# yuliangguo/OmniFusion

Measured on AMD Instinct MI355X. Metric: panoramas/sec at 512x1024 ERP, N=18 256^2 patches; equi2pers+pers2equi GB/s vs HBM peak, higher is better.
Workload: dtype f16x3 (fp16 hi/lo pairs, fp32 accumulate: fp32-class); 1 GPU; cfg2/cfg4 shard: 8 panoramas/GPU/step, 512x1024 ERP, fov 80, nrows 4 (18 patches); full single-pass spherical_fusion forward (confidence=True) at patch size 128 — the only size the reference network exists at (SURVEY 0.1); random-init weights (seed 42); inputs resident in HBM; resample pair at 18x256^2 reported in roofline_resample; per_gpu_batch=8, global_batch=8, parallelism=image-sharded x1, execution=3 forwards in flight per GPU on 3 streams (spherical_fusion.pipelined)

## Files before the change

omnifusion_amd/csrc/omni_conv_up2_taps.hip:

```cpp
#include <stdint.h>
#include "omni_up2_tapsum.h"

namespace {

struct TapsArgs {
    const void* src;
    const void* wt;
    const float* bias;
    void* dst;
    int M, Hl, Cout, act;
};

constexpr int TAP_BYTES = 32 * 256;

__device__ __forceinline__ void wait_taps_in_flight(int n)
{
    if (n >= 16) wait_vm<16>();
    else if (n == 14) wait_vm<14>();
    else if (n == 12) wait_vm<12>();
    else if (n == 10) wait_vm<10>();
    else if (n == 8) wait_vm<8>();
    else if (n == 6) wait_vm<6>();
    else if (n == 4) wait_vm<4>();
    else if (n == 2) wait_vm<2>();
    else wait_vm<0>();
}

template <int WL, int ROWS, int HALO>
__global__ __launch_bounds__(256, 1) void up2_taps_fused_kernel(TapsArgs a)
{
    static_assert((WL == 32 && ROWS == 8 && HALO == 1) || (WL == 16 && ROWS == 16 && HALO == 0), "bands of 8 rows of 32-wide maps, or whole 16 x 16 maps");
    constexpr int SROWS = ROWS + 2 * HALO, P = SROWS * WL, NF = P / 32, NFW = (NF + 3) / 4;
    constexpr int W_BYTES = 9 * TAP_BYTES, CH_BYTES = P * 128, ROW_BYTES = WL * 128;
    static_assert(P % 32 == 0 && ROWS * WL == 256, "whole fragments; one (column, channel quad) thread per eight rows");
    __shared__ __attribute__((aligned(1024))) unsigned char lds[W_BYTES + 2 * CH_BYTES];
    static_assert(sizeof(lds) <= 160 * 1024, "one block per CU");

    const int t = threadIdx.x, lane = t & 63;
    const int wave = __builtin_amdgcn_readfirstlane(t >> 6);
    const int ntn = a.Cout >> 5, nb = a.Hl / ROWS;
    int bid = blockIdx.x;
    const int tile_n = bid % ntn; bid /= ntn;
    const int band = bid % nb; const int m = bid / nb;
    const int r0 = band * ROWS, col0 = tile_n * 32, sbase = r0 - HALO;
    const int Hl = a.Hl;

    auto frag = [&](int fi) { const int f = wave + 4 * fi; return f < NF ? f : wave + 4; };
    h8v xh[NFW][4], xl[NFW][4];
#pragma unroll
    for (int fi = 0; fi < NFW; ++fi) {
        const int f = frag(fi);
        {
            const int p = f * 32 + (lane & 31), sr = p / WL, cx = p - sr * WL;
            const int row = min(max(sbase + sr, 0), Hl - 1);
            const unsigned char* sp = (const unsigned char*)a.src + ((size_t)(m * Hl + row) * WL + cx) * 256 + (lane >> 5) * 16;
#pragma unroll
            for (int kc = 0; kc < 4; ++kc) {
                xh[fi][kc] = *reinterpret_cast<const h8v*>(sp + (kc >> 1) * 128 + (kc & 1) * 32);
                xl[fi][kc] = *reinterpret_cast<const h8v*>(sp + (kc >> 1) * 128 + 64 + (kc & 1) * 32);
            }
        }
    }
    {
        const rsrc_t rsw = make_rsrc(a.wt, (size_t)9 * a.Cout * 256);
#pragma unroll
        for (int s = 0; s < 9; ++s) {
            const int tp = tap_at(s);
#pragma unroll
            for (int k = 0; k < 2; ++k) {
                const int i = wave + 4 * k, row = 4 * i + (lane >> 4), piece = (lane & 15) ^ (row & 15);
                dma16(rsw, lds + tp * TAP_BYTES + i * 1024, ((tp * a.Cout + col0 + row) * 16 + piece) * 16, 0);
            }
        }
    }
    const int wfo = (lane & 31) * 256 + (((lane >> 5) ^ (lane & 15)) * 16);

    const int quad = t & 7, j = (t >> 3) & (WL - 1);
    const int ib = WL == 32 ? 0 : 8 * (wave >> 1);
    int coff[3];
#pragma unroll
    for (int c = 0; c < 3; ++c) coff[c] = tapsum_col_off(min(max(j - 1 + c, 0), WL - 1), quad);
    float hx[4], lx[4];
    tapsum_col_weights<WL>(j, hx, lx);
    const TapsumRowW wy = tapsum_row_weights(r0 + ib == 0, r0 + ib + 7 == Hl - 1);

    f4v out[8][2][2];
    f4v S[8][2];

    wait_taps_in_flight(16);
    __builtin_amdgcn_s_barrier();
    asm volatile("" ::: "memory");

    auto tap = [&]<int s>() {
        constexpr int tp = tap_at(s), ky = tp / 3, kx = tp - 3 * ky;
        unsigned char* chunk = lds + W_BYTES + (s & 1) * CH_BYTES;
        {
            const unsigned char* wb = lds + tp * TAP_BYTES;
            h8v wh[4], wl[4];
#pragma unroll
            for (int kc = 0; kc < 4; ++kc) {
                const int K = 8 * (kc >> 1) + 2 * (kc & 1);
                wh[kc] = *reinterpret_cast<const h8v*>(wb + (wfo ^ (K * 16)));
                wl[kc] = *reinterpret_cast<const h8v*>(wb + (wfo ^ ((K + 4) * 16)));
            }
#pragma unroll
            for (int fi = 0; fi < NFW; ++fi) {
                const int f = frag(fi);
                {
                    f16v acc = (f16v)(0.0f), acc1 = (f16v)(0.0f);
#pragma unroll
                    for (int kc = 0; kc < 4; ++kc) {
                        acc  = __builtin_amdgcn_mfma_f32_32x32x16_f16(wh[kc], xh[fi][kc], acc, 0, 0, 0);
                        acc1 = __builtin_amdgcn_mfma_f32_32x32x16_f16(wl[kc], xh[fi][kc], acc1, 0, 0, 0);
                        acc1 = __builtin_amdgcn_mfma_f32_32x32x16_f16(wh[kc], xl[fi][kc], acc1, 0, 0, 0);
                    }
                    const int px = f * 32 + (lane & 31);
                    tapsum_park(acc1, acc, chunk + px * 128, (px >> 1) & 3, lane >> 5);
                }
                __builtin_amdgcn_sched_barrier(0);
            }
        }
        if (s < 8) wait_taps_in_flight(2 * (7 - s));
        wait_lds_reads();
        __builtin_amdgcn_s_barrier();
        asm volatile("" ::: "memory");
        tapsum_vertical<8, ky, ROW_BYTES>(S, chunk, r0 + ib, sbase, Hl, coff[1], wy);
        if constexpr (ky == 2) {
            unsigned char* other = lds + W_BYTES + ((s & 1) ^ 1) * CH_BYTES;
            tapsum_put<8, 0, ROW_BYTES>(S, other, ib, coff[1]);
            wait_lds_reads();
            __builtin_amdgcn_s_barrier();
            asm volatile("" ::: "memory");
            tapsum_put<8, 1, ROW_BYTES>(S, chunk, ib, coff[1]);
            __builtin_amdgcn_sched_barrier(0);
            tapsum_horizontal<8, kx, 0, ROW_BYTES>(out, S, other, ib, coff[0], coff[2], hx, lx);
            wait_lds_reads();
            __builtin_amdgcn_s_barrier();
            asm volatile("" ::: "memory");
            tapsum_horizontal<8, kx, 1, ROW_BYTES>(out, S, chunk, ib, coff[0], coff[2], hx, lx);
        }
    };
    tap.template operator()<0>(); tap.template operator()<1>(); tap.template operator()<2>();
    tap.template operator()<3>(); tap.template operator()<4>(); tap.template operator()<5>();
    tap.template operator()<6>(); tap.template operator()<7>(); tap.template operator()<8>();

    f4v bv = (f4v)(0.0f);
    if (a.bias) bv = *reinterpret_cast<const f4v*>(a.bias + col0 + quad * 4);
    const int Ho = 2 * Hl, Wo = 2 * WL;
#pragma unroll
    for (int it = 0; it < 8; ++it)
#pragma unroll
        for (int ay = 0; ay < 2; ++ay)
#pragma unroll
            for (int bx = 0; bx < 2; ++bx) {
                f4v o = out[it][ay][bx] + bv;
                if (a.act == OMNI_ACT_RELU) { o.x = fmaxf(o.x, 0.f); o.y = fmaxf(o.y, 0.f); o.z = fmaxf(o.z, 0.f); o.w = fmaxf(o.w, 0.f); }
                const int oy = 2 * (r0 + ib + it) + ay, ox = 2 * j + bx;
                act_store4<true>(a.dst, (((size_t)m * Ho + oy) * Wo + ox) * a.Cout + col0 + quad * 4, o);
            }
}

}

OMNI_SH_OVERFLOW_ACCESSOR(omni_sh_overflow_up2_taps)

extern "C" int omni_conv3x3_up2_taps_sh_f16x3(const void* src, const void* wt16t, const float* bias, void* dst, int fmt,
                                              int M, int Hl, int Wl, int C, int Cout, int act, omni_stream_t stream)
{
    if (!src || !wt16t || !dst) OMNI_FAIL(OMNI_ERR_INVALID, "omni_conv3x3_up2_taps_sh: null pointer");
    if (M <= 0 || Hl <= 0 || Wl <= 0 || C <= 0 || C % 32 || Cout <= 0 || Cout % 32) OMNI_FAIL(OMNI_ERR_INVALID, "omni_conv3x3_up2_taps_sh: bad shape (channels must be multiples of 32)");
    if ((uintptr_t)src % 16 || (uintptr_t)wt16t % 16 || (uintptr_t)bias % 16 || (uintptr_t)dst % 16) OMNI_FAIL(OMNI_ERR_INVALID, "omni_conv3x3_up2_taps_sh: tensors must be 16-byte aligned");
    const bool bands = Wl == 32 && Hl % 8 == 0, image = Wl == 16 && Hl == 16;
    if ((fmt & ~4) != 1 || C != 64 || Cout != 64 || !(bands || image) || (act != OMNI_ACT_NONE && act != OMNI_ACT_RELU))
        OMNI_FAIL(OMNI_ERR_UNSUPPORTED, "omni_conv3x3_up2_taps_sh: serves f16x3 with an SH result, 64 -> 64 channels, Wl = 32 with Hl % 8 == 0 or 16 x 16 maps, no activation or ReLU");
    if ((long long)M * Hl * Wl * 4 >= (1ll << 31)) OMNI_FAIL(OMNI_ERR_UNSUPPORTED, "omni_conv3x3_up2_taps_sh: tensor too large for 32-bit indices");
    TapsArgs a;
    a.src = src; a.wt = wt16t; a.bias = bias; a.dst = dst; a.M = M; a.Hl = Hl; a.Cout = Cout; a.act = act;
    const unsigned ntn = (unsigned)(Cout / 32);
    if (bands) hipLaunchKernelGGL((up2_taps_fused_kernel<32, 8, 1>), dim3((unsigned)M * (unsigned)(Hl / 8) * ntn), dim3(256), 0, (hipStream_t)stream, a);
    else       hipLaunchKernelGGL((up2_taps_fused_kernel<16, 16, 0>), dim3((unsigned)M * ntn), dim3(256), 0, (hipStream_t)stream, a);
    OMNI_HIP(hipGetLastError());
    return OMNI_OK;
}
```

omnifusion_amd/csrc/omni_geometry.hip:

```cpp
#include <math.h>
#include <stdlib.h>
#include <string.h>
#include <mutex>
#include <vector>
#include <memory>

#include "omni_internal.h"

static thread_local std::string g_err;
void omni_set_error(const std::string& msg) { g_err = msg; }
extern "C" const char* omni_last_error(void) { return g_err.c_str(); }
extern "C" int omni_version(void) { return OMNI_VERSION; }

namespace {
struct OptName { const char* name; const char* env; int OmniOptions::* field; int dflt; };
const OptName kOpts[] = {
    {"conv_sh_tile", "OMNI_CONV_SH_TILE", &OmniOptions::conv_sh_tile, -1},
    {"conv_nohalo", "OMNI_CONV_NOHALO", &OmniOptions::conv_nohalo, 0},
    {"conv_halo_th", "OMNI_CONV_HALO_TH", &OmniOptions::conv_halo_th, 4},
    {"conv_big_blocks", "OMNI_CONV_BIG_BLOCKS", &OmniOptions::conv_big_blocks, 128},
    {"conv_halo_bn_lat", "OMNI_CONV_HALO_BN_LAT", &OmniOptions::conv_halo_bn_lat, 32},
    {"conv_deep_loaders", "OMNI_CONV_DEEP_LOADERS", &OmniOptions::conv_deep_loaders, 1},
    {"conv_halo_up2_bn_lat", "OMNI_CONV_HALO_UP2_BN_LAT", &OmniOptions::conv_halo_up2_bn_lat, 64},
    {"conv_halo_bn", "OMNI_CONV_HALO_BN", &OmniOptions::conv_halo_bn, 64},
    {"conv_img", "OMNI_CONV_IMG", &OmniOptions::conv_img, 1},
    {"conv_nodeep", "OMNI_CONV_NODEEP", &OmniOptions::conv_nodeep, 0},
    {"conv_pingpong", "OMNI_CONV_PINGPONG", &OmniOptions::conv_pingpong, 1},
    {"conv_pm", "OMNI_CONV_PM", &OmniOptions::conv_pm, 1},
    {"conv_noxcd", "OMNI_CONV_NOXCD", &OmniOptions::conv_noxcd, 0},
    {"conv_wt_major", "OMNI_CONV_WT_MAJOR", &OmniOptions::conv_wt_major, 1},
    {"conv_stem_pc", "OMNI_CONV_STEM_PC", &OmniOptions::conv_stem_pc, 1},
    {"conv_epi_lds", "OMNI_CONV_EPI_LDS", &OmniOptions::conv_epi_lds, 1},
    {"conv_up2_persist", "OMNI_CONV_UP2_PERSIST", &OmniOptions::conv_up2_persist, 1},
    {"conv_up2_heads_taps", "OMNI_CONV_UP2_HEADS_TAPS", &OmniOptions::conv_up2_heads_taps, 1},
    {"splitk_max", "OMNI_SPLITK_MAX", &OmniOptions::splitk_max, 0},
    {"e2p_gather", "OMNI_E2P_GATHER", &OmniOptions::e2p_gather, 0},
    {"e2p_notab", "OMNI_E2P_NOTAB", &OmniOptions::e2p_notab, 0},
    {"e2p_verbose", "OMNI_E2P_VERBOSE", &OmniOptions::e2p_verbose, 0},
    {"e2p_bwd_simple", "OMNI_E2P_BWD_SIMPLE", &OmniOptions::e2p_bwd_simple, 0},
    {"p2e_bwd_simple", "OMNI_P2E_BWD_SIMPLE", &OmniOptions::p2e_bwd_simple, 0},
    {"bwd_table_mb", "OMNI_BWD_TABLE_MB", &OmniOptions::bwd_table_mb, 1024},
    {"bwd_wide", "OMNI_BWD_WIDE", &OmniOptions::bwd_wide, 1},
    {"bwd_lmax", "OMNI_BWD_LMAX", &OmniOptions::bwd_lmax, 0},
    {"bwd_chunk", "OMNI_BWD_CHUNK", &OmniOptions::bwd_chunk, 0},
    {"p2e_gather", "OMNI_P2E_GATHER", &OmniOptions::p2e_gather, 0},
    {"e2p_nbuf", "OMNI_E2P_NBUF", &OmniOptions::e2p_nbuf, 0},
    {"e2p_slot_kb", "OMNI_E2P_SLOT_KB", &OmniOptions::e2p_slot_kb, 6},
    {"e2p_tile_h", "OMNI_E2P_TILE_H", &OmniOptions::e2p_tile_h, 0},
    {"e2p_ref_lds", "OMNI_E2P_REF_LDS", &OmniOptions::e2p_ref_lds, 1},
    {"e2p_store", "OMNI_E2P_STORE", &OmniOptions::e2p_store, 1},
    {"e2p_slots", "OMNI_E2P_SLOTS", &OmniOptions::e2p_slots, 0},
    {"e2p_split", "OMNI_E2P_SPLIT", &OmniOptions::e2p_split, 0},
    {"e2p_full", "OMNI_E2P_FULL", &OmniOptions::e2p_full, -1},
    {"e2p_fb_planes", "OMNI_E2P_FB_PLANES", &OmniOptions::e2p_fb_planes, 0},
    {"e2p_fb_pos", "OMNI_E2P_FB_POS", &OmniOptions::e2p_fb_pos, 0},
    {"e2p_region", "OMNI_E2P_REGION", &OmniOptions::e2p_region, 0},
    {"p2e_band", "OMNI_P2E_BAND", &OmniOptions::p2e_band, 0},
    {"p2e_nbuf", "OMNI_P2E_NBUF", &OmniOptions::p2e_nbuf, 0},
    {"p2e_lds_kb", "OMNI_P2E_LDS_KB", &OmniOptions::p2e_lds_kb, 0},
    {"p2e_planes", "OMNI_P2E_PLANES", &OmniOptions::p2e_planes, 0},
    {"p2e_walk", "OMNI_P2E_WALK", &OmniOptions::p2e_walk, 1},
    {"p2e_tile8", "OMNI_P2E_TILE8", &OmniOptions::p2e_tile8, 1},
    {"p2e_store", "OMNI_P2E_STORE", &OmniOptions::p2e_store, 1},
    {"fv_bwd_lds", "OMNI_FV_BWD_LDS", &OmniOptions::fv_bwd_lds, 1},
    {"geom_cache_max", "OMNI_GEOM_CACHE_MAX", &OmniOptions::geom_cache_max, 16},
    {"chamfer_split", "OMNI_CHAMFER_SPLIT", &OmniOptions::chamfer_split, 1},
    {"augment_lut", "OMNI_AUGMENT_LUT", &OmniOptions::augment_lut, 1},
    {"conv_halo2", "OMNI_CONV_HALO2", &OmniOptions::conv_halo2, 1},
    {"conv_wgrad_rows", "OMNI_CONV_WGRAD_ROWS", &OmniOptions::conv_wgrad_rows, 0},
};
}

OmniOptions& omni_options()
{
    static OmniOptions o = [] {
        OmniOptions v;
        for (const OptName& k : kOpts) {
            const char* e = getenv(k.env);
            v.*(k.field) = e ? (*e ? atoi(e) : 1) : k.dflt;
        }
        return v;
    }();
    return o;
}

int omni_num_cus()
{
    static int cus[64] = {0};
    int dev = 0;
    if (hipGetDevice(&dev) != hipSuccess || dev < 0 || dev >= 64) return 256;
    if (cus[dev] == 0) {
        int n = 0;
        cus[dev] = (hipDeviceGetAttribute(&n, hipDeviceAttributeMultiprocessorCount, dev) == hipSuccess && n > 0) ? n : 256;
    }
    return cus[dev];
}

extern "C" int omni_set_option(const char* name, int value)
{
    if (!name) OMNI_FAIL(OMNI_ERR_INVALID, "omni_set_option: null name");
    for (const OptName& k : kOpts)
        if (strcmp(k.name, name) == 0) { omni_options().*(k.field) = value; return OMNI_OK; }
    OMNI_FAIL(OMNI_ERR_INVALID, std::string("omni_set_option: unknown option '") + name + "'");
}

extern "C" int omni_get_option(const char* name, int* value)
{
    if (!name || !value) OMNI_FAIL(OMNI_ERR_INVALID, "omni_get_option: null argument");
    for (const OptName& k : kOpts)
        if (strcmp(k.name, name) == 0) { *value = omni_options().*(k.field); return OMNI_OK; }
    OMNI_FAIL(OMNI_ERR_INVALID, std::string("omni_get_option: unknown option '") + name + "'");
}

#ifdef OMNI_DEBUG_BUILD
int omni_debug_bits(const char* env_name) { const char* d = getenv(env_name); return d ? atoi(d) : 0; }
static long long* g_omni_trace = nullptr;
long long* omni_debug_trace_buf() { return g_omni_trace; }
extern "C" int omni_debug_set_trace(long long* buf) { g_omni_trace = buf; return OMNI_OK; }
#endif

namespace {
struct Preset { int nr; const int* cols; const double* phis; };

bool preset(int nrows, int which, Preset& p)
{
    static const int c4[] = {3, 6, 6, 3};            static const double p4[] = {-67.5, -22.5, 22.5, 67.5};
    static const int c6[] = {3, 8, 12, 12, 8, 3};    static const double p6[] = {-75.2, -45.93, -15.72, 15.72, 45.93, 75.2};
    static const int c3[] = {3, 4, 3};               static const double p3e[] = {-60, 0, 60};
    static const double p3p[] = {-59.6, 0, 59.6};
    static const int c5[] = {3, 6, 8, 6, 3};         static const double p5[] = {-72.2, -36.1, 0, 36.1, 72.2};
    switch (nrows) {
    case 4: p = {4, c4, p4}; return true;
    case 6: p = {6, c6, p6}; return true;
    case 3: p = {3, c3, which ? p3p : p3e}; return true;
    case 5: p = {5, c5, p5}; return true;
    default: return false;
    }
}

int centers(int nrows, int which, float* lam0, float* phi1, float* center_p)
{
    Preset p;
    if (!preset(nrows, which, p)) return -1;
    const float PI_F = (float)M_PI, PI_2_F = (float)(M_PI * 0.5);
    int n = 0;
    for (int i = 0; i < p.nr; ++i)
        for (int j = 0; j < p.cols[i]; ++j) {
            double ti = 360.0 / p.cols[i];
            double tc = j * ti + ti / 2;
            float cx = (float)tc / 360.0f;
            float cy = ((float)p.phis[i] + 90.0f) / 180.0f;
            float px = cx * 2.0f - 1.0f, py = cy * 2.0f - 1.0f;
            if (center_p) { center_p[2 * n] = px; center_p[2 * n + 1] = py; }
            if (lam0) lam0[n] = px * PI_F;
            if (phi1) phi1[n] = py * PI_2_F;
            ++n;
        }
    return n;
}

void fill_tab(PatchTab& t, int nrows, int which)
{
    float lam[OMNI_MAX_PATCH], phi[OMNI_MAX_PATCH];
    t.N = centers(nrows, which, lam, phi, nullptr);
    for (int n = 0; n < t.N; ++n) {
        t.lam0[n] = lam[n];
        t.slam[n] = (float)sin((double)lam[n]); t.clam[n] = (float)cos((double)lam[n]);
        t.sphi[n] = (float)sin((double)phi[n]); t.cphi[n] = (float)cos((double)phi[n]);
    }
}

float linspace_f(float start, float end, int steps, int idx)
{
    if (steps == 1) return start;
    float step = (end - start) / (float)(steps - 1);
    int half = steps / 2;
    return idx < half ? fmaf(step, (float)idx, start) : fmaf(-step, (float)(steps - idx - 1), end);
}
}

extern "C" int omni_num_patches(int nrows) { return centers(nrows, 0, nullptr, nullptr, nullptr); }

extern "C" int omni_patch_centers(int nrows, int which, float* center_p_host)
{
    if (!center_p_host) OMNI_FAIL(OMNI_ERR_INVALID, "omni_patch_centers: null output");
    int n = centers(nrows, which, nullptr, nullptr, center_p_host);
    if (n < 0) OMNI_FAIL(OMNI_ERR_INVALID, "unsupported nrows " + std::to_string(nrows) + " (presets: 3,4,5,6)");
    return OMNI_OK;
}

extern "C" int omni_geometry_create(omni_geometry_t** out, int nrows, float fov_h, float fov_w,
                                    int ph, int pw, int H, int W, omni_stream_t stream_)
{
    hipStream_t stream = (hipStream_t)stream_;
    if (!out) OMNI_FAIL(OMNI_ERR_INVALID, "omni_geometry_create: null out");
    if (omni_num_patches(nrows) < 0)
        OMNI_FAIL(OMNI_ERR_INVALID, "unsupported nrows " + std::to_string(nrows) + " (presets: 3,4,5,6)");
    if (ph < 1 || pw < 1 || H < 0 || W < 0 || ph > 32768 || pw > 32768 || H > 32768 || W > 32768)
        OMNI_FAIL(OMNI_ERR_INVALID, "omni_geometry_create: bad patch/ERP size");
    if (!(fov_h > 0.f) || !(fov_w > 0.f)) OMNI_FAIL(OMNI_ERR_INVALID, "omni_geometry_create: fov must be > 0");

    std::unique_ptr<omni_geometry> g(new omni_geometry());
    OMNI_HIP(hipGetDevice(&g->device));
    g->nrows = nrows; g->fov_h = fov_h; g->fov_w = fov_w; g->ph = ph; g->pw = pw; g->H = H; g->W = W;
    fill_tab(g->e2p, nrows, 0);
    fill_tab(g->p2e, nrows, 1);
    g->N = g->e2p.N;
    centers(nrows, 0, nullptr, nullptr, g->center_p);
    g->row_trig = nullptr; g->col_trig = nullptr; g->cand = nullptr; g->ntx = (W + 63) / 64;
    g->e2p_fb_tiles = nullptr; g->e2p_nfb = 0; g->e2p_ixy = nullptr; g->e2p_ts = 32;
    for (auto& t : g->p2e_tiles) { t.ent = nullptr; t.ord = nullptr; t.walk = nullptr; t.nslots = 0; t.max_chunks = 0; t.max_cand = 0; t.ok = 0; t.sum_chunks = 0; }
    for (auto& t : g->e2p_boxes) { t.ent = nullptr; t.fb = nullptr; t.order = nullptr; t.norder = 0; t.nfb = 0; t.max_chunks = 0; t.ok = 0; t.tw = t.th = t.tx = t.ty = 0; }
    g->p2e_tx = g->p2e_ty = 0; g->pinned = 0;
    g->p2e_bwd_box = nullptr; g->p2e_rden = nullptr; g->p2e_btx = g->p2e_bty = g->p2e_bwd_ok = 0;
    g->p2e_bwd_ids = nullptr; g->p2e_bwd_nsmall = g->p2e_bwd_nbig = 0;
    g->e2p_bwd_box = nullptr; g->e2p_bwd_ids = nullptr; g->e2p_bwd_nsmall = g->e2p_bwd_nbig = g->e2p_gtx = g->e2p_gty = g->e2p_bwd_ok = 0;

    if (H > 0 && W > 0) {
        const float PI_F = (float)M_PI, PI_2_F = (float)(M_PI * 0.5);
        std::vector<float2> rt(H), ct(W);
        for (int i = 0; i < H; ++i) { double a = (double)linspace_f(-PI_2_F, PI_2_F, H, i); rt[i] = make_float2((float)sin(a), (float)cos(a)); }
        for (int j = 0; j < W; ++j) { double a = (double)linspace_f(-PI_F, PI_F, W, j);     ct[j] = make_float2((float)sin(a), (float)cos(a)); }
        OMNI_HIP(hipMalloc((void**)&g->row_trig, sizeof(float2) * H));
        OMNI_HIP(hipMalloc((void**)&g->col_trig, sizeof(float2) * W));
        OMNI_HIP(hipMalloc((void**)&g->cand, sizeof(unsigned long long) * (size_t)H * g->ntx));
        OMNI_HIP(hipMemcpy(g->row_trig, rt.data(), sizeof(float2) * H, hipMemcpyHostToDevice));
        OMNI_HIP(hipMemcpy(g->col_trig, ct.data(), sizeof(float2) * W, hipMemcpyHostToDevice));
        int rc = omni_p2e_build_candidates(g.get(), stream);
        if (rc == OMNI_OK) rc = omni_p2e_build_tiles(g.get(), stream);
        if (rc == OMNI_OK) rc = omni_e2p_build_tileflags(g.get(), stream);
        if (rc == OMNI_OK) rc = omni_e2p_build_boxes(g.get(), stream);
        if (rc != OMNI_OK) { omni_geometry_destroy(g.release()); return rc; }
    }
    *out = g.release();
    return OMNI_OK;
}

int omni_bwd_workspace(omni_geometry* g, hipStream_t stream, size_t bytes, float** out)
{
    std::lock_guard<std::mutex> lk(g->ws_mu);
    omni_geometry::Ws* w = nullptr;
    for (auto& x : g->bwd_ws)
        if (x.stream == stream) {
            if (x.bytes >= bytes) { *out = x.ptr; return OMNI_OK; }
            w = &x;
        }
    hipStreamCaptureStatus cs = hipStreamCaptureStatusNone;
    if (stream && hipStreamIsCapturing(stream, &cs) == hipSuccess && cs == hipStreamCaptureStatusActive)
        OMNI_FAIL(OMNI_ERR_UNSUPPORTED, "backward: first use of a batch size on this geometry and stream while the stream is being captured (run the shape once before capturing)");
    if (!w || g->pinned) { g->bwd_ws.push_back({stream, nullptr, 0}); w = &g->bwd_ws.back(); }
    if (w->ptr) { OMNI_HIP(hipStreamSynchronize(stream)); OMNI_HIP(hipFree(w->ptr)); w->ptr = nullptr; w->bytes = 0; }
    OMNI_HIP(hipMalloc((void**)&w->ptr, bytes));
    w->bytes = bytes; *out = w->ptr;
    return OMNI_OK;
}

extern "C" void omni_geometry_destroy(omni_geometry_t* g)
{
    if (!g) return;
    if (g->row_trig) (void)hipFree(g->row_trig);
    if (g->col_trig) (void)hipFree(g->col_trig);
    if (g->cand) (void)hipFree(g->cand);
    for (auto& t : g->p2e_tiles) { if (t.ent) (void)hipFree(t.ent); if (t.ord) (void)hipFree(t.ord); if (t.walk) (void)hipFree(t.walk); }
    if (g->p2e_bwd_box) (void)hipFree(g->p2e_bwd_box);
    if (g->p2e_rden) (void)hipFree(g->p2e_rden);
    if (g->p2e_bwd_ids) (void)hipFree(g->p2e_bwd_ids);
    for (auto& t : g->e2p_boxes) { if (t.ent) (void)hipFree(t.ent); if (t.fb) (void)hipFree(t.fb); if (t.order) (void)hipFree(t.order); for (auto& w : t.work) (void)hipFree(w.dev); }
    if (g->e2p_fb_tiles) (void)hipFree(g->e2p_fb_tiles);
    if (g->e2p_ixy) (void)hipFree(g->e2p_ixy);
    if (g->e2p_bwd_box) (void)hipFree(g->e2p_bwd_box);
    if (g->e2p_bwd_ids) (void)hipFree(g->e2p_bwd_ids);
    omni_sp_free(g->p2e_sp); omni_sp_free(g->e2p_sp);
    for (auto& w : g->bwd_ws) if (w.ptr) (void)hipFree(w.ptr);
    delete g;
}

namespace {
std::mutex g_mu;
std::vector<omni_geometry*> g_cache;

void destroy_drained(omni_geometry* g)
{
    int cur = 0;
    if (hipGetDevice(&cur) == hipSuccess) {
        if (cur != g->device) (void)hipSetDevice(g->device);
        (void)hipDeviceSynchronize();
        if (cur != g->device) (void)hipSetDevice(cur);
    }
    omni_geometry_destroy(g);
}
}

int omni_geometry_lookup(const omni_geometry** out, int nrows, float fov_h, float fov_w,
                         int ph, int pw, int H, int W, hipStream_t stream)
{
    int dev = 0;
    OMNI_HIP(hipGetDevice(&dev));
    std::lock_guard<std::mutex> lk(g_mu);
    for (size_t i = 0; i < g_cache.size(); ++i) {
        omni_geometry* g = g_cache[i];
        if (g->device == dev && g->nrows == nrows && g->fov_h == fov_h && g->fov_w == fov_w &&
            g->ph == ph && g->pw == pw && g->H == H && g->W == W) {
            if (i) { g_cache.erase(g_cache.begin() + i); g_cache.insert(g_cache.begin(), g); }
            hipStreamCaptureStatus cs = hipStreamCaptureStatusNone;
            if (stream && hipStreamIsCapturing(stream, &cs) == hipSuccess && cs == hipStreamCaptureStatusActive) g->pinned = 1;
            *out = g; return OMNI_OK;
        }
    }
    {
        hipStreamCaptureStatus cs = hipStreamCaptureStatusNone;
        if (stream && hipStreamIsCapturing(stream, &cs) == hipSuccess && cs == hipStreamCaptureStatusActive)
            OMNI_FAIL(OMNI_ERR_UNSUPPORTED, "omni_geometry_lookup: first use of a geometry while its stream is being captured (run the shape once before capturing)");
    }
    omni_geometry* g = nullptr;
    int rc = omni_geometry_create(&g, nrows, fov_h, fov_w, ph, pw, H, W, stream);
    if (rc != OMNI_OK) return rc;
    g_cache.insert(g_cache.begin(), g);
    const size_t cap = (size_t)(omni_options().geom_cache_max > 0 ? omni_options().geom_cache_max : 1);
    for (size_t i = g_cache.size(); i-- > 1 && g_cache.size() > cap;)
        if (!g_cache[i]->pinned) { destroy_drained(g_cache[i]); g_cache.erase(g_cache.begin() + i); }
    *out = g;
    return OMNI_OK;
}

extern "C" int omni_geometry_cache_size(void)
{
    std::lock_guard<std::mutex> lk(g_mu);
    return (int)g_cache.size();
}

extern "C" void omni_geometry_cache_clear(void)
{
    std::lock_guard<std::mutex> lk(g_mu);
    for (omni_geometry* g : g_cache) destroy_drained(g);
    g_cache.clear();
}
```

omnifusion_amd/csrc/omni_internal.h:

```cpp
#pragma once
#include <mutex>
#include <hip/hip_runtime.h>
#include <hip/hip_fp16.h>
#include <stdint.h>
#include <string>
#include <vector>

#include "../../include/omnifusion.h"

#define OMNI_MAX_PATCH 46
#define OMNI_WAVE 64

void omni_set_error(const std::string& msg);
#define OMNI_FAIL(code, msg) do { omni_set_error(msg); return (code); } while (0)
#define OMNI_HIP(expr) do { hipError_t e_ = (expr); if (e_ != hipSuccess) {                   \
        omni_set_error(std::string(#expr) + ": " + hipGetErrorString(e_)); return OMNI_ERR_HIP; } } while (0)

struct OmniOptions {
    int conv_sh_tile;
    int conv_nohalo;
    int conv_halo_th;
    int conv_halo_bn_lat;
    int conv_halo_up2_bn_lat;
    int conv_deep_loaders;
    int conv_big_blocks;
    int conv_halo_bn;
    int conv_img;
    int conv_nodeep;
    int conv_pingpong;
    int conv_pm;
    int conv_noxcd;
    int conv_wt_major;
    int conv_stem_pc;
    int conv_epi_lds;
    int conv_up2_persist;
    int conv_up2_heads_taps;
    int splitk_max;
    int e2p_gather;
    int e2p_notab;
    int e2p_verbose;
    int e2p_bwd_simple;
    int p2e_bwd_simple;
    int p2e_gather;
    int e2p_nbuf;
    int e2p_store;
    int e2p_slots;
    int e2p_split;
    int e2p_full;
    int e2p_fb_planes;
    int e2p_region;
    int e2p_fb_pos;
    int e2p_ref_lds;
    int e2p_tile_h;
    int e2p_slot_kb;
    int p2e_band;
    int p2e_lds_kb;
    int p2e_nbuf;
    int p2e_planes;
    int p2e_store;
    int p2e_tile8;
    int p2e_walk;
    int bwd_wide;
    int bwd_chunk;
    int bwd_lmax;
    int bwd_table_mb;
    int fv_bwd_lds;
    int geom_cache_max;
    int chamfer_split;
    int augment_lut;
    int conv_halo2;
    int conv_wgrad_rows;
};
OmniOptions& omni_options();
int omni_num_cus();

#ifdef OMNI_DEBUG_BUILD
#define OMNI_DBG(a, bit) (((a).dbg & (bit)) != 0)
int omni_debug_bits(const char* env_name);
long long* omni_debug_trace_buf();
#else
#define OMNI_DBG(a, bit) false
#endif

struct PatchTab {
    int   N;
    float lam0[OMNI_MAX_PATCH];
    float slam[OMNI_MAX_PATCH];
    float clam[OMNI_MAX_PATCH];
    float sphi[OMNI_MAX_PATCH];
    float cphi[OMNI_MAX_PATCH];
};

constexpr int OMNI_SP_LMAX = 48;
struct OmniSpTable {
    uint2* ent = nullptr; int* slice_off = nullptr; int* cnt = nullptr;
    uint2* long_ent = nullptr; int* long_off = nullptr; int* long_row = nullptr;
    int nrows = 0, nslices = 0, nlong = 0, ok = 0;
    long long nent = 0, npadded = 0, nlong_ent = 0;
};
void omni_sp_free(OmniSpTable& t);
struct omni_geometry;
int omni_bwd_workspace(omni_geometry* g, hipStream_t stream, size_t bytes, float** out);

struct omni_geometry {
    int device;
    int pinned;
    int nrows, N;
    float fov_h, fov_w;
    int ph, pw, H, W;
    PatchTab e2p;
    PatchTab p2e;
    float center_p[2 * OMNI_MAX_PATCH];
    float2* row_trig;
    float2* col_trig;
    unsigned long long* cand;
    int ntx;
    struct P2ETiles { uint2* ent; int max_chunks; int max_cand; int ok; int sum_chunks; uint2* ord; int nslots; unsigned char* walk; int nslots_walk; } p2e_tiles[4];
    int p2e_tx, p2e_ty;
    int4* p2e_bwd_box; float* p2e_rden; int p2e_btx, p2e_bty, p2e_bwd_ok;
    int* p2e_bwd_ids; int p2e_bwd_nsmall, p2e_bwd_nbig;
    struct E2PWorkTab { long long key; uint4* dev; int nblocks; };
    struct E2PTiles { uint2* ent; int* fb; int nfb; int max_chunks; int tw, th, tx, ty; int ok;
                      int* order; int norder;
                      std::vector<uint2> h_ent; std::vector<int> h_order, h_fb, h_region;
                      std::vector<E2PWorkTab> work; } e2p_boxes[2];
    std::mutex work_mu;
    int* e2p_fb_tiles;
    int e2p_nfb;
    int e2p_ts;
    float2* e2p_ixy;
    int4* e2p_bwd_box; int* e2p_bwd_ids; int e2p_bwd_nsmall, e2p_bwd_nbig, e2p_gtx, e2p_gty, e2p_bwd_ok;
    OmniSpTable p2e_sp, e2p_sp;
    struct Ws { hipStream_t stream; float* ptr; size_t bytes; };
    std::vector<Ws> bwd_ws; std::mutex ws_mu;
    std::mutex bwd_mu; int p2e_bwd_tried = 0, e2p_bwd_tried = 0;
};

int omni_geometry_lookup(const omni_geometry** out, int nrows, float fov_h, float fov_w,
                         int ph, int pw, int H, int W, hipStream_t stream);
int omni_p2e_build_candidates(omni_geometry* g, hipStream_t stream);
int omni_p2e_build_tiles(omni_geometry* g, hipStream_t stream);
int omni_p2e_build_bwd(omni_geometry* g, hipStream_t stream);
int omni_e2p_build_tileflags(omni_geometry* g, hipStream_t stream);
int omni_e2p_build_boxes(omni_geometry* g, hipStream_t stream);
int omni_e2p_build_bwd(omni_geometry* g, hipStream_t stream);

template <typename T> struct Store;
template <> struct Store<float> {
    static __device__ __forceinline__ float ld(const float* p) { return *p; }
    static __device__ __forceinline__ void st(float* p, float v) { *p = v; }
    static __device__ __forceinline__ void st_nt(float* p, float v) { __builtin_nontemporal_store(v, p); }
};
template <> struct Store<__half> {
    static __device__ __forceinline__ float ld(const __half* p) { return __half2float(*p); }
    static __device__ __forceinline__ void st(__half* p, float v) { *p = __float2half_rn(v); }
    static __device__ __forceinline__ void st_nt(__half* p, float v)
    { const __half h = __float2half_rn(v); __builtin_nontemporal_store(*reinterpret_cast<const unsigned short*>(&h), reinterpret_cast<unsigned short*>(p)); }
};

__device__ __forceinline__ unsigned omni_xcd_remap(unsigned bid, unsigned nblocks)
{
    const unsigned per = nblocks >> 3;
    const unsigned full = per << 3;
    if (bid >= full) return bid;
    return (bid & 7u) * per + (bid >> 3);
}

__host__ __device__ inline int omni_xcd_band_rows(int rows) { const int b = rows / 16; return b < 1 ? 1 : (b > 8 ? 8 : b); }
__host__ __device__ inline int omni_xcd_rows_grid(int rows, int cols)
{
    const int band = omni_xcd_band_rows(rows);
    return 8 * ((rows + 8 * band - 1) / (8 * band)) * band * cols;
}
__device__ __forceinline__ bool omni_xcd_rows(unsigned bid, int rows, int cols, int& row, int& col)
{
    const int band = omni_xcd_band_rows(rows);
    const unsigned x = bid & 7u, k = bid >> 3, per = (unsigned)(band * cols);
    const unsigned bl = k / per, wi = k - bl * per;
    row = (int)((bl * 8u + x) * (unsigned)band + wi / (unsigned)cols);
    col = (int)(wi % (unsigned)cols);
    return row < rows;
}
```

omnifusion_amd/isa.py:

```python
import os
import re
import subprocess
import sys
import tempfile

LLVM = os.environ.get("OMNI_LLVM_BIN", "/opt/rocm/lib/llvm/bin")
TARGET = "hipv4-amdgcn-amd-amdhsa--gfx950"
FORBIDDEN = re.compile(r"\bv_pk_(mul|add|fma)_f32\b")
COUNTED = ("e2p_box_kernel", "p2e_lds_kernel", "p2e_walk_kernel", "e2p_ref_kernel", "up2_taps_fused_kernel", "up2_heads_taps_kernel")
HOT = ("conv_sh_kernel", "conv3x3_halo_sh_kernel", "conv3x3_up2_g1_kernel", "stem_f16x3_pc_kernel", "heads_kernel", "maxpool_kernel",
       "layernorm512_kernel", "attention_kernel", "upsample_sh8_kernel", "halo2_sh_kernel")
HOST_ONLY = ("omni_png.o", "omni_geometry.o")


def _device_object(obj, tmp):
    fat = os.path.join(tmp, "fat.bin")
    co = os.path.join(tmp, "dev.co")
    r = subprocess.run([os.path.join(LLVM, "llvm-objcopy"), "--dump-section", f".hip_fatbin={fat}", obj, os.path.join(tmp, "copy.o")],
                       stderr=subprocess.DEVNULL)
    if r.returncode != 0 or not os.path.exists(fat) or os.path.getsize(fat) == 0:
        return None
    subprocess.check_call([os.path.join(LLVM, "clang-offload-bundler"), "--unbundle", "--type=o", f"--input={fat}",
                           f"--targets={TARGET}", f"--output={co}"])
    return co


def disassemble(obj):
    with tempfile.TemporaryDirectory() as tmp:
        co = _device_object(obj, tmp)
        if co is None:
            return ""
        return subprocess.check_output([os.path.join(LLVM, "llvm-objdump"), "-d", "--mcpu=gfx950", co]).decode()


def kernel_meta(obj):
    with tempfile.TemporaryDirectory() as tmp:
        co = _device_object(obj, tmp)
        if co is None:
            return []
        txt = subprocess.check_output([os.path.join(LLVM, "llvm-readelf"), "--notes", co]).decode()
    out, cur = [], None
    keys = {".vgpr_count": "vgpr", ".agpr_count": "agpr", ".sgpr_count": "sgpr", ".group_segment_fixed_size": "lds",
            ".private_segment_fixed_size": "scratch", ".vgpr_spill_count": "vgpr_spill", ".sgpr_spill_count": "sgpr_spill",
            ".name": "name"}
    for line in txt.splitlines():
        m = re.match(r"^  - \.(\w+):\s*(\S+)\s*$", line)
        if m:
            cur = {}
            out.append(cur)
            line = "    ." + m.group(1) + ": " + m.group(2)
        m = re.match(r"^    (\.\w+):\s*(\S+)\s*$", line)
        if m and cur is not None and m.group(1) in keys:
            v = m.group(2)
            cur[keys[m.group(1)]] = v if m.group(1) == ".name" else int(v)
    return [k for k in out if "name" in k]


def demangle(names):
    try:
        p = subprocess.run([os.path.join(LLVM, "llvm-cxxfilt")], input="\n".join(names).encode(), stdout=subprocess.PIPE, check=True)
        return p.stdout.decode().splitlines()
    except Exception:
        return list(names)


def objects():
    from . import build as b
    return [s[:-4] + ".o" for s in b.sources()]


def check(objs=None):
    bad = []
    found = {c: 0 for c in COUNTED + HOT}
    full = objs is None
    for obj in objs or objects():
        base = os.path.basename(obj)
        if not os.path.exists(obj):
            bad.append(f"{base}: object missing (build first)")
            continue
        asm = disassemble(obj)
        if not asm.strip():
            if base not in HOST_ONLY:
                bad.append(f"{base}: no gfx950 device code could be extracted (not in HOST_ONLY): the ISA rules were NOT checked")
            continue
        cur = "?"
        for line in asm.splitlines():
            if line.endswith(">:"):
                cur = line.split("<", 1)[1][:-2]
            elif FORBIDDEN.search(line):
                bad.append(f"{base}: packed-fp32 instruction in {cur}: {line.strip()[:80]}")
                break
        for k in kernel_meta(obj):
            for c in COUNTED + HOT:
                if c in k["name"]:
                    found[c] += 1
            if any(c in k["name"] for c in COUNTED):
                if k.get("scratch", 0) or k.get("vgpr_spill", 0):
                    bad.append(f"{base}: {k['name']} uses scratch {k.get('scratch')} B / spills {k.get('vgpr_spill')} VGPR "
                               f"{k.get('sgpr_spill')} SGPR — its hand-counted s_waitcnt vmcnt(N) would be off")
            elif any(c in k["name"] for c in HOT):
                if k.get("scratch", 0) or k.get("vgpr_spill", 0):
                    bad.append(f"{base}: {k['name']} (a kernel with >= 1 % of the bench's GPU time) uses scratch {k.get('scratch')} B / "
                               f"spills {k.get('vgpr_spill')} VGPR")
    if full:
        for c, n in found.items():
            if n == 0:
                bad.append(f"guarded kernel `{c}` was not found in any code object's metadata: the scratch rule for it was NOT checked")
    return bad


def table(objs=None):
    rows = []
    for obj in objs or objects():
        meta = kernel_meta(obj)
        for k, nm in zip(meta, demangle([k["name"] for k in meta])):
            nm = nm.replace("(anonymous namespace)::", "")
            nm = re.sub(r"\(.*$", "", nm)
            rows.append((os.path.basename(obj), nm, k.get("vgpr", 0), k.get("agpr", 0), k.get("sgpr", 0), k.get("lds", 0), k.get("scratch", 0)))
    return rows


if __name__ == "__main__":
    if "--check" in sys.argv:
        v = check()
        for line in v:
            print("ISA CHECK FAILED:", line)
        print("isa check:", "FAILED" if v else "ok (no v_pk_*_f32; counted-wait and hot kernels without scratch; every guarded kernel found)")
        sys.exit(1 if v else 0)
    print(f"{'object':22s} {'vgpr':>4s} {'agpr':>4s} {'sgpr':>4s} {'lds':>6s} {'scr':>4s}  kernel")
    for o, nm, v, a, s, l, sc in table():
        print(f"{o:22s} {v:4d} {a:4d} {s:4d} {l:6d} {sc:4d}  {nm[:150]}")
```

Baseline: 4539 panoramas/s.

## Add persistent XCD-partitioned walk kernel for the up2 taps-fused convolution

Adds a persistent 512-thread kernel that walks (band, Cout-half) work units assigned per XCD. It reloads weights only when the Cout half changes and prefetches the next unit's input fragments during the last tap. Each thread now covers four rows instead of eight, which lowers per-thread accumulator pressure and doubles the waves per block. It is enabled by default for the banded case and meant to cut per-block launch and weight-reload overhead and improve latency hiding. The trade-offs are hardcoded Cout=64, more complex counted waits, and serialized work within each CU.

Measured after the change: 4593 panoramas/s (median of 6 runs). 1.01x the previous value.

```diff
diff --git a/omnifusion_amd/csrc/omni_conv_up2_taps.hip b/omnifusion_amd/csrc/omni_conv_up2_taps.hip
--- a/omnifusion_amd/csrc/omni_conv_up2_taps.hip
+++ b/omnifusion_amd/csrc/omni_conv_up2_taps.hip
@@ -1,4 +1,5 @@
 #include <stdint.h>
+#include <algorithm>
 #include "omni_up2_tapsum.h"
 
 namespace {
@@ -160,6 +161,174 @@
             }
 }
 
+struct WalkArgs {
+    const void* src;
+    const void* wt;
+    const float* bias;
+    void* dst;
+    int Hl, act, npairs;
+};
+
+template <int WL>
+__global__ __launch_bounds__(512, 1) void up2_taps_walk_kernel(WalkArgs a)
+{
+    static_assert(WL == 32 || WL == 16, "bands of 8 rows of 32-wide maps, or whole 16 x 16 maps");
+    constexpr int BROWS = WL == 32 ? 8 : 16, HALO = WL == 32 ? 1 : 0, ROWS = 4;
+    constexpr int SROWS = BROWS + 2 * HALO, P = SROWS * WL, NF = P / 32, NFW = (NF + 7) / 8;
+    constexpr int W_BYTES = 9 * TAP_BYTES, CH_BYTES = P * 128, ROW_BYTES = WL * 128;
+    static_assert(P % 32 == 0 && BROWS * WL * 8 == 512 * ROWS && NF <= 16, "whole fragments; one (column, channel quad, row group) thread per four rows");
+    __shared__ __attribute__((aligned(1024))) unsigned char lds[W_BYTES + 2 * CH_BYTES];
+    static_assert(sizeof(lds) <= 160 * 1024 && BROWS * ROW_BYTES <= CH_BYTES, "one block per CU; one ay half of the vertical sums fits a chunk");
+
+    const int t = threadIdx.x, lane = t & 63;
+    const int wave = __builtin_amdgcn_readfirstlane(t >> 6);
+    const int Hl = a.Hl, nb = Hl / BROWS;
+    const int xcd = blockIdx.x & 7, lb = blockIdx.x >> 3, nlb = gridDim.x >> 3;
+    const int per = (a.npairs + 7) >> 3, u_end = 2 * min(a.npairs, (xcd + 1) * per);
+    int u = 2 * xcd * per + lb;
+    if (u >= u_end) return;
+    int half = u & 1;
+
+    auto frag = [&](int fi) { return fi == 0 || wave + 8 >= NF ? wave : wave + 8; };
+    h8v xh[NFW][4], xl[NFW][4];
+    auto load_x = [&](int unit) {
+        const int pr = unit >> 1, m = pr / nb, sbase = (pr - m * nb) * BROWS - HALO;
+#pragma unroll
+        for (int fi = 0; fi < NFW; ++fi) {
+            const int p = frag(fi) * 32 + (lane & 31), sr = p / WL, cx = p - sr * WL;
+            const int row = min(max(sbase + sr, 0), Hl - 1);
+            const unsigned char* sp = (const unsigned char*)a.src + ((size_t)(m * Hl + row) * WL + cx) * 256 + (lane >> 5) * 16;
+#pragma unroll
+            for (int kc = 0; kc < 4; ++kc) {
+                xh[fi][kc] = *reinterpret_cast<const h8v*>(sp + (kc >> 1) * 128 + (kc & 1) * 32);
+                xl[fi][kc] = *reinterpret_cast<const h8v*>(sp + (kc >> 1) * 128 + 64 + (kc & 1) * 32);
+            }
+        }
+    };
+    const rsrc_t rsw = make_rsrc(a.wt, (size_t)9 * 64 * 256);
+    auto load_w = [&](int h) {
+#pragma unroll
+        for (int s = 0; s < 9; ++s) {
+            const int tp = tap_at(s), row = 4 * wave + (lane >> 4), piece = (lane & 15) ^ (row & 15);
+            dma16(rsw, lds + tp * TAP_BYTES + wave * 1024, ((tp * 64 + h * 32 + row) * 16 + piece) * 16, 0);
+        }
+    };
+    load_x(u);
+    load_w(half);
+    const int wfo = (lane & 31) * 256 + (((lane >> 5) ^ (lane & 15)) * 16);
+
+    const int quad = t & 7, j = (t >> 3) & (WL - 1);
+    const int ib = ROWS * (wave / (WL / 8));
+    const int coff1 = tapsum_col_off(j, quad);
+    bool first = true;
+
+    wait_vm<8>();
+    __builtin_amdgcn_s_barrier();
+    asm volatile("" ::: "memory");
+
+    for (;;) {
+        const int pr = u >> 1, m = pr / nb, band = pr - m * nb;
+        const int r0 = band * BROWS, sbase = r0 - HALO;
+        const int col0 = half * 32;
+        const int next = u + nlb;
+        const TapsumRowW wy = tapsum_row_weights(r0 + ib == 0, r0 + ib + ROWS - 1 == Hl - 1);
+
+        f4v out[ROWS][2][2];
+        f4v S[ROWS][2];
+
+        auto tap = [&]<int s>() {
+            constexpr int tp = tap_at(s), ky = tp / 3, kx = tp - 3 * ky;
+            unsigned char* chunk = lds + W_BYTES + (s & 1) * CH_BYTES;
+            {
+                const unsigned char* wb = lds + tp * TAP_BYTES;
+                int ln = lane, wf = wfo;
+                asm volatile("" : "+v"(ln), "+v"(wf));
+#pragma unroll
+                for (int fi = 0; fi < NFW; ++fi) {
+                    if (fi == 1 && wave + 8 >= NF) break;
+                    f16v acc = (f16v)(0.0f), acc1 = (f16v)(0.0f);
+#pragma unroll
+                    for (int kh = 0; kh < 2; ++kh) {
+                        h8v wh[2], wl[2];
+#pragma unroll
+                        for (int k2 = 0; k2 < 2; ++k2) {
+                            const int K = 8 * kh + 2 * k2;
+                            wh[k2] = *reinterpret_cast<const h8v*>(wb + (wf ^ (K * 16)));
+                            wl[k2] = *reinterpret_cast<const h8v*>(wb + (wf ^ ((K + 4) * 16)));
+                        }
+#pragma unroll
+                        for (int k2 = 0; k2 < 2; ++k2) {
+                            const int kc = 2 * kh + k2;
+                            acc  = __builtin_amdgcn_mfma_f32_32x32x16_f16(wh[k2], xh[fi][kc], acc, 0, 0, 0);
+                            acc1 = __builtin_amdgcn_mfma_f32_32x32x16_f16(wl[k2], xh[fi][kc], acc1, 0, 0, 0);
+                            acc1 = __builtin_amdgcn_mfma_f32_32x32x16_f16(wh[k2], xl[fi][kc], acc1, 0, 0, 0);
+                        }
+                    }
+                    const int px = frag(fi) * 32 + (ln & 31);
+                    tapsum_park(acc1, acc, chunk + px * 128, (px >> 1) & 3, ln >> 5);
+                    __builtin_amdgcn_sched_barrier(0);
+                }
+            }
+            if constexpr (s < 8) { if (first) wait_vm<7 - s>(); }
+            else load_x(next < u_end ? next : u);
+            wait_lds_reads();
+            __builtin_amdgcn_s_barrier();
+            asm volatile("" ::: "memory");
+            tapsum_vertical<ROWS, ky, ROW_BYTES>(S, chunk, r0 + ib, sbase, Hl, coff1, wy);
+            if constexpr (ky == 2) {
+                unsigned char* other = lds + W_BYTES + ((s & 1) ^ 1) * CH_BYTES;
+                auto horizontal = [&]<int ay>(const unsigned char* buf) {
+                    int jj = j;
+                    asm volatile("" : "+v"(jj));
+                    float hx[4], lx[4];
+                    tapsum_col_weights<WL>(jj, hx, lx);
+                    tapsum_horizontal<ROWS, kx, ay, ROW_BYTES>(out, S, buf, ib, tapsum_col_off(max(jj - 1, 0), quad), tapsum_col_off(min(jj + 1, WL - 1), quad), hx, lx);
+                };
+                tapsum_put<ROWS, 0, ROW_BYTES>(S, other, ib, coff1);
+                wait_lds_reads();
+                __builtin_amdgcn_s_barrier();
+                asm volatile("" ::: "memory");
+                tapsum_put<ROWS, 1, ROW_BYTES>(S, chunk, ib, coff1);
+                __builtin_amdgcn_sched_barrier(0);
+                horizontal.template operator()<0>(other);
+                wait_lds_reads();
+                __builtin_amdgcn_s_barrier();
+                asm volatile("" ::: "memory");
+                horizontal.template operator()<1>(chunk);
+            }
+        };
+        tap.template operator()<0>(); tap.template operator()<1>(); tap.template operator()<2>();
+        tap.template operator()<3>(); tap.template operator()<4>(); tap.template operator()<5>();
+        tap.template operator()<6>(); tap.template operator()<7>(); tap.template operator()<8>();
+
+        f4v bv = (f4v)(0.0f);
+        if (a.bias) bv = *reinterpret_cast<const f4v*>(a.bias + col0 + quad * 4);
+        const int Ho = 2 * Hl, Wo = 2 * WL;
+#pragma unroll
+        for (int it = 0; it < ROWS; ++it)
+#pragma unroll
+            for (int ay = 0; ay < 2; ++ay)
+#pragma unroll
+                for (int bx = 0; bx < 2; ++bx) {
+                    f4v o = out[it][ay][bx] + bv;
+                    if (a.act == OMNI_ACT_RELU) { o.x = fmaxf(o.x, 0.f); o.y = fmaxf(o.y, 0.f); o.z = fmaxf(o.z, 0.f); o.w = fmaxf(o.w, 0.f); }
+                    const int oy = 2 * (r0 + ib + it) + ay, ox = 2 * j + bx;
+                    act_store4<true>(a.dst, (((size_t)m * Ho + oy) * Wo + ox) * 64 + col0 + quad * 4, o);
+                }
+        if (next >= u_end) break;
+        u = next;
+        first = false;
+        if ((u & 1) != half) {
+            half = u & 1;
+            load_w(half);
+            wait_vm<0>();
+        }
+        wait_lds_reads();
+        __builtin_amdgcn_s_barrier();
+        asm volatile("" ::: "memory");
+    }
+}
+
 }
 
 OMNI_SH_OVERFLOW_ACCESSOR(omni_sh_overflow_up2_taps)
@@ -176,6 +345,21 @@
     if ((long long)M * Hl * Wl * 4 >= (1ll << 31)) OMNI_FAIL(OMNI_ERR_UNSUPPORTED, "omni_conv3x3_up2_taps_sh: tensor too large for 32-bit indices");
     TapsArgs a;
     a.src = src; a.wt = wt16t; a.bias = bias; a.dst = dst; a.M = M; a.Hl = Hl; a.Cout = Cout; a.act = act;
+    constexpr bool WALK_BANDS = true, WALK_IMAGE = false;
+    const OmniOptions& o = omni_options();
+    const int wk = o.conv_up2_taps_walk;
+    if (bands ? (wk == 1 && WALK_BANDS) || wk == 2 || wk == 3 : (wk == 1 && WALK_IMAGE) || wk == 2 || wk == 4) {
+        WalkArgs k;
+        k.src = src; k.wt = wt16t; k.bias = bias; k.dst = dst; k.Hl = Hl; k.act = act; k.npairs = bands ? M * (Hl / 8) : M;
+        const long long units = 2ll * k.npairs;
+        const int cus = std::max(8, omni_num_cus() / 8 * 8);
+        long long grid = units < cus ? (units + 7) / 8 * 8 : cus;
+        if (o.conv_up2_taps_walk_grid > 0) grid = std::min<long long>(grid, std::max(8, o.conv_up2_taps_walk_grid / 8 * 8));
+        if (bands) hipLaunchKernelGGL(up2_taps_walk_kernel<32>, dim3((unsigned)grid), dim3(512), 0, (hipStream_t)stream, k);
+        else       hipLaunchKernelGGL(up2_taps_walk_kernel<16>, dim3((unsigned)grid), dim3(512), 0, (hipStream_t)stream, k);
+        OMNI_HIP(hipGetLastError());
+        return OMNI_OK;
+    }
     const unsigned ntn = (unsigned)(Cout / 32);
     if (bands) hipLaunchKernelGGL((up2_taps_fused_kernel<32, 8, 1>), dim3((unsigned)M * (unsigned)(Hl / 8) * ntn), dim3(256), 0, (hipStream_t)stream, a);
     else       hipLaunchKernelGGL((up2_taps_fused_kernel<16, 16, 0>), dim3((unsigned)M * ntn), dim3(256), 0, (hipStream_t)stream, a);
diff --git a/omnifusion_amd/csrc/omni_geometry.hip b/omnifusion_amd/csrc/omni_geometry.hip
--- a/omnifusion_amd/csrc/omni_geometry.hip
+++ b/omnifusion_amd/csrc/omni_geometry.hip
@@ -33,6 +33,8 @@
     {"conv_epi_lds", "OMNI_CONV_EPI_LDS", &OmniOptions::conv_epi_lds, 1},
     {"conv_up2_persist", "OMNI_CONV_UP2_PERSIST", &OmniOptions::conv_up2_persist, 1},
     {"conv_up2_heads_taps", "OMNI_CONV_UP2_HEADS_TAPS", &OmniOptions::conv_up2_heads_taps, 1},
+    {"conv_up2_taps_walk", "OMNI_CONV_UP2_TAPS_WALK", &OmniOptions::conv_up2_taps_walk, 1},
+    {"conv_up2_taps_walk_grid", "OMNI_CONV_UP2_TAPS_WALK_GRID", &OmniOptions::conv_up2_taps_walk_grid, 0},
     {"splitk_max", "OMNI_SPLITK_MAX", &OmniOptions::splitk_max, 0},
     {"e2p_gather", "OMNI_E2P_GATHER", &OmniOptions::e2p_gather, 0},
     {"e2p_notab", "OMNI_E2P_NOTAB", &OmniOptions::e2p_notab, 0},
diff --git a/omnifusion_amd/csrc/omni_internal.h b/omnifusion_amd/csrc/omni_internal.h
--- a/omnifusion_amd/csrc/omni_internal.h
+++ b/omnifusion_amd/csrc/omni_internal.h
@@ -35,6 +35,8 @@
     int conv_epi_lds;
     int conv_up2_persist;
     int conv_up2_heads_taps;
+    int conv_up2_taps_walk;
+    int conv_up2_taps_walk_grid;
     int splitk_max;
     int e2p_gather;
     int e2p_notab;
diff --git a/omnifusion_amd/isa.py b/omnifusion_amd/isa.py
--- a/omnifusion_amd/isa.py
+++ b/omnifusion_amd/isa.py
@@ -7,7 +7,7 @@
 LLVM = os.environ.get("OMNI_LLVM_BIN", "/opt/rocm/lib/llvm/bin")
 TARGET = "hipv4-amdgcn-amd-amdhsa--gfx950"
 FORBIDDEN = re.compile(r"\bv_pk_(mul|add|fma)_f32\b")
-COUNTED = ("e2p_box_kernel", "p2e_lds_kernel", "p2e_walk_kernel", "e2p_ref_kernel", "up2_taps_fused_kernel", "up2_heads_taps_kernel")
+COUNTED = ("e2p_box_kernel", "p2e_lds_kernel", "p2e_walk_kernel", "e2p_ref_kernel", "up2_taps_fused_kernel", "up2_heads_taps_kernel", "up2_taps_walk_kernel")
 HOT = ("conv_sh_kernel", "conv3x3_halo_sh_kernel", "conv3x3_up2_g1_kernel", "stem_f16x3_pc_kernel", "heads_kernel", "maxpool_kernel",
        "layernorm512_kernel", "attention_kernel", "upsample_sh8_kernel", "halo2_sh_kernel")
 HOST_ONLY = ("omni_png.o", "omni_geometry.o")
```
